# VinAIResearch/DiMSUM

Measured on AMD Instinct MI355X. Metric: denoiser-fwd latents/sec, higher is better.
Workload: dtype f32; 1 GPU; DiM-L/2 denoiser forward, 256px (4x32x32 latents, 256 tokens), 256 latents per GPU, random-init weights (reference init, zero tensors re-drawn N(0, 0.02^2)); global_batch=256, parallelism=dp1 (replicas, independent latents), launch=eager, matmul_policy=f16s (see notes.matmul_policy)

## Files before the change

### dimsum_amd/csrc/gemm_nt.hip

```cpp
#include "gemm_nt_kernel.hpp"

namespace dimsum {
namespace gemm_nt {

struct gemm_flat_t : dimsum_gemm_ext_t {
    int32_t m, n, k, operand_dtype, epilogue;
    float out_scale;
    int64_t lda, ldb, ldc;
    const void *a_ptr, *b_ptr, *bias_ptr;
    void *c_ptr;
    const void *a_inv_scale_ptr, *b_inv_scale_ptr;
};
static int gemm_flat_from(const dimsum_gemm_params_t *p, gemm_flat_t &f) {
    if (!p) return DIMSUM_ERR_NULL;
    if (p->struct_size != sizeof(dimsum_gemm_params_t)) return DIMSUM_ERR_ABI;
    const int rc = ext_from<dimsum_gemm_ext_t>(p->ext, f);
    if (rc != DIMSUM_OK) return rc;
    f.m = p->m; f.n = p->n; f.k = p->k; f.operand_dtype = p->operand_dtype; f.epilogue = p->epilogue; f.out_scale = p->out_scale;
    f.lda = p->lda; f.ldb = p->ldb; f.ldc = p->ldc;
    f.a_ptr = p->a_ptr; f.b_ptr = p->b_ptr; f.bias_ptr = p->bias_ptr; f.c_ptr = p->c_ptr;
    f.a_inv_scale_ptr = p->a_inv_scale_ptr; f.b_inv_scale_ptr = p->b_inv_scale_ptr;
    return DIMSUM_OK;
}

// ... 69 lines not shown
    if (w.probe) { *w.probe = 1; return DIMSUM_OK; }
    Args a = a0;
    a.tiles_m = a.M / 128;
    a.group_m = a.tiles_m <= 32 ? a.tiles_m : 2 * a0.group_m;
    return run<gemm_nt_m128_kernel<kOp, kEpi, kVar>>(a, a.tiles_m * a.tiles_n, 256, w);
}
inline int persist_grid() {
    int dev = 0, cus = 256;
    if (hipGetDevice(&dev) == hipSuccess) (void)hipDeviceGetAttribute(&cus, hipDeviceAttributeMultiprocessorCount, dev);
    return cus >= 8 ? cus / 8 * 8 : 8;
}
template <int kOp, int kEpi, int kVar = 0> int launch_persist(const Args &a, const Where &w) {
    if (w.probe) { *w.probe = 2; return DIMSUM_OK; }
    return run<gemm_nt_persist_kernel<kOp, kEpi, kVar>>(a, persist_grid(), 512, w);
}
template <int kEpi, int kVar = 0> int launch_f16(const Args &a, const Where &w, bool m128) {
    return m128 ? launch_m128<kOpF16, kEpi, kVar>(a, w) : launch<kOpF16, kEpi, kVar>(a, w);
}

inline bool m128_tiles(int epilogue, bool bf, int k, int tune_variant) {
    if (bf || epilogue == DIMSUM_GEMM_EPI_GATED_GELU_SPLIT3) return false;
    if (tune_variant != 0) return tune_variant == 512;
    switch (epilogue) {
        case DIMSUM_GEMM_EPI_F32: case DIMSUM_GEMM_EPI_F32_BIAS: case DIMSUM_GEMM_EPI_F16_QKV: case DIMSUM_GEMM_EPI_F32_CONV: return k <= 576;
        default: return false;
    }
}
inline bool persist_ok(const Args &a, int epilogue, bool bf, int tune_variant) {
    const bool gated = epilogue == DIMSUM_GEMM_EPI_GATED_GELU_F16;
    if (bf || tune_variant == 512 || tune_variant == 513 || !(gated || (epilogue == DIMSUM_GEMM_EPI_F32_GATE_RESIDUAL && tune_variant == 514))) return false;
    const int nk = a.K / kBK;
    return a.N % (gated ? 128 : kBN) == 0 && nk >= 4 && nk % 2 == 0 && a.tiles_m * a.tiles_n > persist_grid() && a.a_alias_tiles == 0 && a.b_alias_tiles == 0;
}

}
}

#ifdef DIMSUM_GEMM_TUNE
#define DIMSUM_GEMM_TUNE_VARIANTS(X) X(1) X(2) X(4) X(8) X(12) X(16) X(3) X(40) X(44) X(72) X(104)
#define DIMSUM_GEMM_TUNE_CASE(V) case V: return launch<kOpBf16, kEpiF32, V>(a, w);
#endif

static int gemm_nt_run(const dimsum_gemm_params_t *pub, void *stream, int *probe) {
    using namespace dimsum;
    using namespace dimsum::gemm_nt;
    gemm_flat_t p;
    Args a;
    if (const int rc = gemm_prologue(pub, p, a)) return rc;
    if (p.m <= 0 || p.n <= 0 || p.k < 2 * kBK || p.m % kBM != 0 || p.k % kBK != 0 || p.n % 4 != 0) return DIMSUM_ERR_SHAPE;
    if (p.a_alias_rows != 0 && (p.a_alias_rows < 0 || p.a_alias_rows % kBK != 0 || p.k != 3 * p.a_alias_rows)) return DIMSUM_ERR_SHAPE;
    if (p.b_alias_rows != 0 && (p.b_alias_rows < 0 || p.b_alias_rows % kBK != 0 || p.k != 3 * p.b_alias_rows || (p.epilogue != DIMSUM_GEMM_EPI_F32 && p.epilogue != DIMSUM_GEMM_EPI_F32_CONV))) return DIMSUM_ERR_SHAPE;
    if (!rows_16bit_ok(p.a_ptr, p.lda, p.a_alias_rows ? 2 * p.a_alias_rows : p.k) || !rows_16bit_ok(p.b_ptr, p.ldb, p.b_alias_rows ? 2 * p.b_alias_rows : p.k)) return DIMSUM_ERR_STRIDE;
    if (!offsets_fit(p, false, false)) return DIMSUM_ERR_STRIDE;
    a.K = p.k;
    a.a_alias_tiles = (int)(p.a_alias_rows / kBK);
    a.a_alias_from = a.a_alias_tiles;
    if (p.a_alias_weight_order) {
        if (!p.a_alias_rows) return DIMSUM_ERR_SHAPE;
        a.a_alias_tiles *= 2;
        a.a_alias_from = a.a_alias_tiles;
    }
    a.b_alias_tiles = (int)(p.b_alias_rows / kBK);
    a.stagger = p.tune_reserved > 0 ? p.tune_reserved : 0;
    if ((p.a_inv_scale_ptr == nullptr) != (p.b_inv_scale_ptr == nullptr)) return DIMSUM_ERR_NULL;
    if (a.sb && !aligned_to<char>(a.sb, 16)) return DIMSUM_ERR_STRIDE;
#ifndef DIMSUM_GEMM_TUNE
    if (p.tune_variant != 0 && p.tune_variant != 512 && p.tune_variant != 513 && p.tune_variant != 514) return DIMSUM_ERR_UNSUPPORTED;
#endif
    const bool bf = p.operand_dtype == DIMSUM_BF16;
    if (p.tune_variant == 512 && bf) return DIMSUM_ERR_UNSUPPORTED;
    const bool m128 = m128_tiles(p.epilogue, bf, p.k, p.tune_variant);
    const Where w = where(p, stream, probe);
    constexpr int kShip = kVarFullLineStores | kVarNtStores;
    if (p.epilogue == DIMSUM_GEMM_EPI_F32_GATE_RESIDUAL) {
        if (!p.residual_ptr) return DIMSUM_ERR_NULL;
        if (!rows_f32_out_ok(p) || p.residual_ld % 4 != 0 || p.residual_ld < p.n || !aligned_to<char>(p.residual_ptr, 16) ||
            (p.bias_ptr && !aligned_to<char>(p.bias_ptr, 16)) || (p.gate_ptr && (p.gate_ld % 4 != 0 || !aligned_to<char>(p.gate_ptr, 16))))
            return DIMSUM_ERR_STRIDE;
        if (p.gate_ptr && (p.rows_per_batch <= 0 || p.rows_per_batch % kBM != 0 || p.m % p.rows_per_batch != 0)) return DIMSUM_ERR_SHAPE;
        fill_right(a, p, p.n, kBN);
        a.res = reinterpret_cast<const float *>(p.residual_ptr);
        a.gate = reinterpret_cast<const float *>(p.gate_ptr);
        a.ldr = p.residual_ld; a.ldg = p.gate_ld;
        a.rows_per_batch = p.gate_ptr ? p.rows_per_batch : p.m;
        if (persist_ok(a, p.epilogue, bf, p.tune_variant)) return launch_persist<kOpF16, kEpiF32GateRes, kShip>(a, w);
        return bf ? launch<kOpBf16, kEpiF32GateRes, kShip>(a, w) : launch_f16<kEpiF32GateRes, kShip>(a, w, m128);
    }
    if (p.epilogue == DIMSUM_GEMM_EPI_F16_QKV) {
        if (bf || !a.sa || !p.gate_bound_ptr) return DIMSUM_ERR_NULL;
        if (p.rows_per_batch <= 0 || p.rows_per_batch % kBM != 0 || p.m % p.rows_per_batch != 0 || p.qkv_q_cols <= 0 || p.qkv_q_cols % 16 != 0 ||
            p.qkv_q_cols > p.n || p.n % 8 != 0)
            return DIMSUM_ERR_SHAPE;
        if (p.ldc % 8 != 0 || p.ldc < p.n || !aligned_to<char>(p.c_ptr, 16) || (p.bias_ptr && !aligned_to<char>(p.bias_ptr, 16)) ||
            (int64_t)257 * p.ldc * 2 >= ((int64_t)1 << 31))
            return DIMSUM_ERR_STRIDE;
        fill_right(a, p, p.n, kBN);
        a.gate_bound = reinterpret_cast<const float *>(p.gate_bound_ptr);
        a.rows_per_batch = p.rows_per_batch;
        a.q_cols = p.qkv_q_cols;
        return launch_f16<kEpiF16Qkv>(a, w, m128);
    }
    if (p.epilogue == DIMSUM_GEMM_EPI_GELU_F16) {
        if (bf || !a.sa || !p.gate_bound_ptr || p.a_alias_rows != 0 || p.x12_ptr || p.c_image_pieces != 0) return DIMSUM_ERR_UNSUPPORTED;
        if (!p.h_inv_scale_ptr) return DIMSUM_ERR_NULL;
        if (p.n % 8 != 0) return DIMSUM_ERR_SHAPE;
        if (p.ldc % 8 != 0 || p.ldc < p.n || !aligned_to<char>(p.c_ptr, 16) || (p.bias_ptr && !aligned_to<char>(p.bias_ptr, 16)) ||
            !aligned_to<char>(p.h_inv_scale_ptr, 4) || (int64_t)257 * p.ldc * 2 >= ((int64_t)1 << 31))
            return DIMSUM_ERR_STRIDE;
        fill_right(a, p, p.n, kBN);
        a.gate_bound = reinterpret_cast<const float *>(p.gate_bound_ptr);
        a.inv_out = reinterpret_cast<float *>(p.h_inv_scale_ptr);
        return launch_f16<kEpiGeluF16>(a, w, m128);
    }
    if (p.epilogue == DIMSUM_GEMM_EPI_F32_CONV) {
        if (!p.conv_weight_ptr) return DIMSUM_ERR_NULL;
        if (p.conv_rows <= 0 || p.conv_rows % kBM != 0 || p.conv_rows > p.m || p.conv_width < 2 || p.conv_width > 4 || p.conv_seq <= 0 || 256 % p.conv_seq != 0 ||
            p.conv_seq % 4 != 0 || p.n % p.conv_seq != 0 || p.conv_weight_ld < p.conv_width)
            return DIMSUM_ERR_SHAPE;
// ... 142 lines not shown
```

### dimsum_amd/csrc/gemm_nt_kernel.hpp

```cpp
#pragma once
#include "common.hpp"

namespace dimsum {
namespace gemm_nt {

typedef float f4 __attribute__((ext_vector_type(4)));
typedef __bf16 bf16x8_t __attribute__((ext_vector_type(8)));
typedef _Float16 f16x8_t __attribute__((ext_vector_type(8)));
typedef unsigned u32x4 __attribute__((ext_vector_type(4)));
typedef unsigned u32x2 __attribute__((ext_vector_type(2)));
typedef __attribute__((address_space(3))) void lds_void_t;
typedef __attribute__((address_space(1))) const void glb_void_t;

constexpr int kBM = 256, kBN = 256, kBK = 64;
constexpr int kHalf = 16384;
constexpr int kParity = 4 * kHalf;
constexpr int kSlotA0 = 0, kSlotA1 = kHalf, kSlotB0 = 2 * kHalf, kSlotB1 = 3 * kHalf;

enum { kOpBf16 = 0, kOpF16 = 1 };
enum { kEpiF32 = 0, kEpiGatedSplit3 = 1, kEpiGatedF16 = 2, kEpiF32Bias = 3, kEpiF32GateRes = 4, kEpiF16Qkv = 5, kEpiF32Conv = 6, kEpiGeluF16 = 7 };

struct Args {
    const char *A, *B0, *B1;
    void *C;
    const float *bias0, *bias1;
    const float *sa, *sb;
    const float *gate_bound;
    float *inv_out;
    const float *res, *gate;
    int64_t ldr, ldg;
    int rows_per_batch;
    int64_t lda, ldb, ldc;
    int M, N, K;
    int tiles_m, tiles_n;
    float out_scale;
    int group_m;
    int stagger;
    float *x12;
    int64_t ldx;
    int splits;
    int64_t c_split_stride;
    int a_alias_tiles;
    int a_alias_from;
    int tn_pieces;
    int64_t a_pair_cols, b_pair_cols;
    int b_alias_tiles;
    const float *conv_w, *conv_b;
    int conv_rows, conv_width, conv_seq, conv_w_ld;
    const float *a_block_inv;
    int a_block_inv_ld;
    const _Float16 *k_fac;
    const float *c_scale;
    const float *k_inv_a, *k_inv_b;
    int q_cols;
    int c_pieces2;
};
enum { kVarLgkmAfterBarrier = 1, kVarNoEpilogue = 2, kVarNtStores = 4, kVarFullLineStores = 8, kVarNoSetprio = 16, kVarSc1Stores = 32, kVarSc0Stores = 64, kVarKeepX12 = 128, kVarTN = 256, kVarM128 = 512, kVarRebase = 1024, kVarPersist = 2048, kVarRowFac = 4096, kVarNN = 8192 };

__device__ __forceinline__ float dpp_row_ror8(float x) {
    const int v = __builtin_bit_cast(int, x);
    return __builtin_bit_cast(float, __builtin_amdgcn_update_dpp(v, v, 0x128, 0xf, 0xf, false));
}
template <int kAux> __device__ __forceinline__ void store_f4(__amdgpu_buffer_rsrc_t rsrc, unsigned voff, const f4 &v) {
    __builtin_amdgcn_raw_buffer_store_b128(__builtin_bit_cast(u32x4, v), rsrc, voff, 0, kAux);
}

template <int kOp> __device__ __forceinline__ f4 mma(const u32x4 &a, const u32x4 &b, f4 c) {
    if constexpr (kOp == kOpBf16) return __builtin_amdgcn_mfma_f32_16x16x32_bf16(__builtin_bit_cast(bf16x8_t, a), __builtin_bit_cast(bf16x8_t, b), c, 0, 0, 0);
    else return __builtin_amdgcn_mfma_f32_16x16x32_f16(__builtin_bit_cast(f16x8_t, a), __builtin_bit_cast(f16x8_t, b), c, 0, 0, 0);
}

__device__ __forceinline__ const char *uniform_ptr(const char *q) {
    const uint64_t v = reinterpret_cast<uint64_t>(q);
    const unsigned lo = __builtin_amdgcn_readfirstlane((unsigned)v), hi = __builtin_amdgcn_readfirstlane((unsigned)(v >> 32));
    return reinterpret_cast<const char *>(((uint64_t)hi << 32) | lo);
}

__device__ __forceinline__ unsigned pick_mask(bool c) {
    unsigned m = c ? 0xffffffffu : 0u;
    asm volatile("" : "+v"(m));
    return m;
}
__device__ __forceinline__ unsigned pick_mask_lanes(bool c) {
    unsigned m = c ? 0xffffffffu : 0u;
    asm volatile("" : "+v"(m));
    return m;
}
__device__ __forceinline__ float pick(unsigned m, float a, float b) {
    return __uint_as_float((__float_as_uint(a) & m) | (__float_as_uint(b) & ~m));
}
__device__ __forceinline__ f4 pick(unsigned m, const f4 &a, const f4 &b) {
    return f4{pick(m, a[0], b[0]), pick(m, a[1], b[1]), pick(m, a[2], b[2]), pick(m, a[3], b[3])};
}

#define DIMSUM_DS_READ_B128(dst, addr, off) asm volatile("ds_read_b128 %0, %1 offset:%2" : "=v"(dst) : "v"(addr), "i"(off))
#define DIMSUM_DS_READ_TR(dst, addr, off) asm volatile("ds_read_b64_tr_b16 %0, %1 offset:%2" : "=v"(dst) : "v"(addr), "i"(off))
#define DIMSUM_WAIT_VM(n) asm volatile("s_waitcnt vmcnt(" #n ")" ::: "memory")
#ifndef DIMSUM_PERSIST_GS
#define DIMSUM_PERSIST_GS 2
#endif
#ifndef DIMSUM_EPI_PACE
#define DIMSUM_EPI_PACE 0
#endif
#define DIMSUM_STR2(x) #x
#define DIMSUM_STR(x) DIMSUM_STR2(x)
#define DIMSUM_PACE_STORES() do { if constexpr (kM1 && DIMSUM_EPI_PACE >= 0) asm volatile("s_waitcnt vmcnt(" DIMSUM_STR(DIMSUM_EPI_PACE) ")" ::: "memory"); } while (0)
#define DIMSUM_WAIT_LGKM0() asm volatile("s_waitcnt lgkmcnt(0)" ::: "memory")

__device__ __forceinline__ float gelu_tanh_f(float x) {
    const float u = 0.7978845608028654f * (x + 0.044715f * x * x * x);
    return x * fast_rcp(1.0f + fast_exp2(-2.0f * kLog2e * u));
}

template <int kOp, int kEpi, int kVar>
__device__ __forceinline__ void gemm_body(const Args &p, char *lds) {
    const unsigned lds0 = (unsigned)(uintptr_t)(__attribute__((address_space(3))) char *)lds;
    const int lane = threadIdx.x & 63;
    const int w = __builtin_amdgcn_readfirstlane(threadIdx.x >> 6);
    constexpr bool kM1 = (kVar & kVarM128) != 0;
    constexpr int kTileM = kM1 ? 128 : kBM;
    constexpr int kMiRows = kM1 ? 64 : 128;
    const int wr = kM1 ? 0 : (w >> 2), wc = w & 3;

    constexpr bool kTN = (kVar & kVarTN) != 0;
    constexpr bool kNN = (kVar & kVarNN) != 0;
    constexpr bool kBT = kTN || kNN;
    static_assert(!kBT || kEpi == kEpiF32, "the TN / NN variants have the plain fp32 epilogue");
    static_assert(!(kBT && kM1) && !(kTN && kNN), "the TN / NN variants have 256 x 256 tiles only");
    constexpr bool kPersist = (kVar & kVarPersist) != 0;
    static_assert(!kPersist || (!kTN && !kM1 && (kEpi == kEpiF32 || kEpi == kEpiF32Bias || kEpi == kEpiF32GateRes || kEpi == kEpiGatedF16)), "persistent: the 256-row NT kernel");
    int tile_m, tile_n, split = 0;
    auto map_tile = [&](int bid, int &tile_m, int &tile_n) {
        const int nwg = kPersist ? p.tiles_m * p.tiles_n : (int)gridDim.x;
        const int q = nwg >> 3, r = nwg & 7, xcd = bid & 7;
        int t = (xcd < r ? xcd * (q + 1) : r * (q + 1) + (xcd - r) * q) + (bid >> 3);
        if constexpr (kBT) {
            const int tiles = p.tiles_m * p.tiles_n;
            split = t / tiles;
            t -= split * tiles;
        }
// ... 78 lines not shown
        tn_b_tile = (int64_t)kBK * p.ldb * 2;
    }
    const unsigned st_lds = lds0 + w * 2048;
    auto stage = [&](int slot, const char *base, unsigned voff, int kt, int alias = 0) {
        const unsigned dst = st_lds + (kt & 1) * kParity + slot;
        const int src_kt = (alias && kt >= (slot < kSlotB0 ? p.a_alias_from : alias)) ? kt - alias : kt;
        const char *s = base + (int64_t)src_kt * (kBK * 2);
        __builtin_amdgcn_global_load_lds((glb_void_t *)(s + voff), (lds_void_t *)(uintptr_t)dst, 16, 0, 0);
        __builtin_amdgcn_global_load_lds((glb_void_t *)(s + 64 + voff), (lds_void_t *)(uintptr_t)(dst + 1024), 16, 0, 0);
    };
    auto stage_tn = [&](int slot, const char *base, int64_t tile_bytes, const unsigned (&voff)[2], int kt) {
        const unsigned dst = st_lds + (kt & 1) * kParity + slot;
        const char *s = base + (int64_t)kt * tile_bytes;
        __builtin_amdgcn_global_load_lds((glb_void_t *)(s + voff[0]), (lds_void_t *)(uintptr_t)dst, 16, 0, 0);
        __builtin_amdgcn_global_load_lds((glb_void_t *)(s + voff[1]), (lds_void_t *)(uintptr_t)(dst + 1024), 16, 0, 0);
    };
    auto stage_tn_a = [&](int slot, const char *base, int kt) {
        const unsigned dst = st_lds + (kt & 1) * kParity + slot;
        const int src_kt = (p.a_alias_tiles && kt >= p.a_alias_tiles) ? kt - p.a_alias_tiles : kt;
        const char *s = base + (int64_t)src_kt * tn_a_tile;
        __builtin_amdgcn_global_load_lds((glb_void_t *)(s + tn_voff_a[0]), (lds_void_t *)(uintptr_t)dst, 16, 0, 0);
        __builtin_amdgcn_global_load_lds((glb_void_t *)(s + tn_voff_a[1]), (lds_void_t *)(uintptr_t)(dst + 1024), 16, 0, 0);
    };
    auto stage_a0 = [&](int kt) { if constexpr (kTN) stage_tn_a(kSlotA0, tn_a, kt); else stage(kSlotA0, a_base, a_voff, kt, p.a_alias_tiles); };
    auto stage_a1 = [&](int kt) { if constexpr (kTN) stage_tn_a(kSlotA1, tn_a + 256, kt); else stage(kSlotA1, a_base + a_half, a_voff, kt, p.a_alias_tiles); };
    auto stage_b0 = [&](int kt) { if constexpr (kBT) stage_tn(kSlotB0, tn_b, tn_b_tile, tn_voff_b, kt); else stage(kSlotB0, b_base[0], b_voff[0], kt, p.b_alias_tiles); };
    auto stage_b1 = [&](int kt) { if constexpr (kBT) stage_tn(kSlotB1, tn_b + 256, tn_b_tile, tn_voff_b, kt); else stage(kSlotB1, b_base[1], b_voff[1], kt, p.b_alias_tiles); };
    auto stage_of = [&](const Src &s_, int which, int kt) {
        if (which == 0) stage(kSlotA0, s_.a_base, a_voff, kt, p.a_alias_tiles);
        else if (which == 1) stage(kSlotB0, s_.b_base[0], s_.b_voff[0], kt, p.b_alias_tiles);
        else if (which == 2) stage(kSlotB1, s_.b_base[1], s_.b_voff[1], kt, p.b_alias_tiles);
        else stage(kSlotA1, s_.a_base + a_half, a_voff, kt, p.a_alias_tiles);
    };

    const unsigned rd = (unsigned)((lane & 15) * 64 + (((lane >> 4) ^ (((lane >> 3) & 1) << 1)) * 16));
    const unsigned a_rd = lds0 + wr * 4 * 2048 + rd;
    const unsigned b_rd = lds0 + wc * 2 * 2048 + rd;

    unsigned a_rd_tn[4], b_rd_tn[2];
    if constexpr (kBT) {
        const int t = lane & 15, g = lane >> 4, key = ((g & 1) << 2) | (t >> 2);
        const unsigned base = lds0 + (unsigned)((4 * g + (t >> 2)) * 256 + (t & 3) * 8);
#pragma unroll
        for (int i = 0; i < 4; ++i) a_rd_tn[i] = base + (unsigned)(((wr * 4 + i) ^ key) << 5);
#pragma unroll
        for (int j = 0; j < 2; ++j) b_rd_tn[j] = base + (unsigned)(((wc * 2 + j) ^ key) << 5);
    }

    u32x4 a0[4][2], a1[4][2], b0[2][2], b1[2][2];
    f4 acc[2][2][4][2];
#pragma unroll
    for (int mi = 0; mi < 2; ++mi)
#pragma unroll
        for (int ni = 0; ni < 2; ++ni)
#pragma unroll
            for (int i = 0; i < 4; ++i)
#pragma unroll
                for (int j = 0; j < 2; ++j) acc[mi][ni][i][j] = f4{0.f, 0.f, 0.f, 0.f};

#define DIMSUM_READ_TN1(dst, addr, slot, kh)                                               \
    do {                                                                                   \
        u32x2 lo_, hi_;                                                                    \
        DIMSUM_DS_READ_TR(lo_, addr, (slot) + (kh) * 8192);                                \
        DIMSUM_DS_READ_TR(hi_, addr, (slot) + (kh) * 8192 + 4096);                         \
        dst = u32x4{lo_[0], lo_[1], hi_[0], hi_[1]};                                       \
    } while (0)
// ... 258 lines not shown
        rebase(a0, 0, (KT) + 1);                     \
        DIMSUM_PHASE_END();                                                                                                     \
    } while (0)
    bool resumed = false;
    for (;;) {
    bool has_next = false;
    int nbid = 0, ntile_m = 0, ntile_n = 0;
    Src nxt = cur;
    if constexpr (kPersist) {
        nbid = bid + (int)gridDim.x;
        has_next = nbid < p.tiles_m * p.tiles_n;
        if (has_next) {
            map_tile(nbid, ntile_m, ntile_n);
            nxt = make_src(ntile_m * kTileM, ntile_n * kTileN);
        }
    }
    if constexpr (kPersist) {
        for (int kt = 0; kt < nk; ++kt) {
            const bool own = kt + 2 < nk;
            const int skt = own ? kt + 2 : kt + 2 - nk;
            Src ss;
            ss.a_base = uniform_ptr(own ? cur.a_base : nxt.a_base);
            ss.b_base[0] = uniform_ptr(own ? cur.b_base[0] : nxt.b_base[0]);
            ss.b_base[1] = uniform_ptr(own ? cur.b_base[1] : nxt.b_base[1]);
            ss.b_voff[0] = cur.b_voff[0];
            ss.b_voff[1] = cur.b_voff[1];
            const bool w12 = !(resumed && kt < 2), w34 = !(resumed && kt < 1);
            DIMSUM_KTILE(kt, stage_of(ss, 0, skt), stage_of(ss, 1, skt), stage_of(ss, 2, skt), stage_of(ss, 3, skt), w12, w34);
        }
        if (wr == 0) __builtin_amdgcn_s_barrier();
    } else if constexpr (!kM1) {
    int kt = 0;
    for (; kt < nk - 2; ++kt) DIMSUM_KTILE(kt, stage_a0(kt + 2), stage_b0(kt + 2), stage_b1(kt + 2), stage_a1(kt + 2), true, true);
    {
        const unsigned par = (kt & 1) * kParity, par_next = kParity - par;
        DIMSUM_READ_B(b0, kSlotB0, par);
        DIMSUM_WAIT_VM(10);
        DIMSUM_PHASE_SYNC();
        DIMSUM_QUADRANT(0, 0, a0, b0);
        DIMSUM_PHASE_END();
        DIMSUM_READ_B(b1, kSlotB1, par);
        DIMSUM_WAIT_VM(8);
        DIMSUM_PHASE_SYNC();
        DIMSUM_QUADRANT(0, 1, a0, b1);
        DIMSUM_PHASE_END();
        DIMSUM_READ_A(a1, kSlotA1, par);
        read_fac(kt);
        DIMSUM_WAIT_VM(6);
        DIMSUM_PHASE_SYNC();
        rebase(a1, 1, kt);
        DIMSUM_QUADRANT(1, 1, a1, b1);
        DIMSUM_PHASE_END();
        DIMSUM_READ_A(a0, kSlotA0, par_next);
        read_fac(kt + 1);
        DIMSUM_WAIT_VM(4);
        DIMSUM_PHASE_SYNC();
        DIMSUM_QUADRANT(1, 0, a1, b0);
        rebase(a0, 0, kt + 1);
        DIMSUM_PHASE_END();
        DIMSUM_READ_B(b0, kSlotB0, par_next);
        DIMSUM_WAIT_VM(2);
        DIMSUM_PHASE_SYNC();
        DIMSUM_QUADRANT(0, 0, a0, b0);
        DIMSUM_PHASE_END();
        DIMSUM_READ_B(b1, kSlotB1, par_next);
        DIMSUM_WAIT_VM(0);
        DIMSUM_PHASE_SYNC();
        DIMSUM_QUADRANT(0, 1, a0, b1);
        DIMSUM_PHASE_END();
        DIMSUM_READ_A(a1, kSlotA1, par_next);
        read_fac(kt + 1);
        DIMSUM_PHASE_SYNC();
        rebase(a1, 1, kt + 1);
        DIMSUM_QUADRANT(1, 1, a1, b1);
        DIMSUM_PHASE_END();
        DIMSUM_QUADRANT(1, 0, a1, b0);
    }
    if (wr == 0) __builtin_amdgcn_s_barrier();
    }

    int lane_e = lane;
    if constexpr (kPersist) asm volatile("" : "+v"(lane_e));
    {
    const int lane = lane_e;
    const int ecol = wc * 32 + (lane >> 4) * 4;
    if constexpr (kVar & kVarNoEpilogue) {
#pragma unroll
        for (int mi = 0; mi < 2; ++mi)
#pragma unroll
            for (int ni = 0; ni < 2; ++ni)
#pragma unroll
                for (int i = 0; i < 4; ++i)
#pragma unroll
                    for (int j = 0; j < 2; ++j) asm volatile("" ::"v"(acc[mi][ni][i][j]));
    } else if constexpr (kEpi == kEpiF32 || kEpi == kEpiF32Bias || kEpi == kEpiF32GateRes || kEpi == kEpiF32Conv) {
        if constexpr (kEpi == kEpiF32Conv) {
            if (m0 < p.conv_rows) {
                constexpr int kNW = kM1 ? 4 : 8;
                constexpr int kHalfRows = kM1 ? 64 : 128;
                float *Ct = reinterpret_cast<float *>(p.C) + (int64_t)m0 * p.ldc + n0;
                const __amdgpu_buffer_rsrc_t crsrc = __builtin_amdgcn_make_buffer_rsrc(Ct, 0, 0x7fffffff, 0x00020000);
                const int W = p.conv_width;
                const bool has_s = p.sa != nullptr;
                const unsigned ms = pick_mask(has_s);
// ... 61 lines not shown
                }
                return;
            }
        }
        constexpr int kAux = ((kVar & kVarNtStores) ? 2 : 0) | ((kVar & kVarSc1Stores) ? 16 : 0) | ((kVar & kVarSc0Stores) ? 1 : 0);
        float *Ct = reinterpret_cast<float *>(p.C) + (int64_t)m0 * p.ldc + n0 + (kBT ? (int64_t)split * p.c_split_stride : (int64_t)0);
        const __amdgpu_buffer_rsrc_t rsrc = __builtin_amdgcn_make_buffer_rsrc(Ct, 0, 0x7fffffff, 0x00020000);
        if constexpr (kVar & kVarFullLineStores) {
            const bool up = (lane & 8) != 0;
            const int frow = wr * 64 + (lane & 7);
            const int fcol = wc * 32 + (lane >> 4) * 4 + (up ? 16 : 0);
            const bool has_s = kRebase || p.sa != nullptr;
            const unsigned ms = pick_mask(has_s);
            const bool has_sb = has_s && !kRowFac;
            const unsigned msb = pick_mask(has_sb);
            const float *sap = p.sa ? p.sa + m0 : reinterpret_cast<const float *>(p.A), *sbp = has_sb ? p.sb : reinterpret_cast<const float *>(p.B0);
            float c_scale = 1.0f;
            if constexpr (kRowFac) c_scale = p.k_inv_a ? c_scale_own : *p.c_scale;
            bool live[2];
            f4 bv[2], sbv[2], gv[2];
            auto load_cols = [&](int ni) {
                const int col = ni * 128 + fcol;
                live[ni] = n0 + col < p.N;
                const int lc = live[ni] ? n0 + col : 0;
                bv[ni] = f4{0.f, 0.f, 0.f, 0.f}; sbv[ni] = gv[ni] = f4{1.f, 1.f, 1.f, 1.f};
                if constexpr (kEpi == kEpiF32Bias) bv[ni] = *reinterpret_cast<const f4 *>(p.bias0 + lc);
                if constexpr (kEpi == kEpiF32GateRes) {
                    bv[ni] = pick(pick_mask(p.bias0 != nullptr), *reinterpret_cast<const f4 *>((p.bias0 ? p.bias0 : reinterpret_cast<const float *>(p.B0)) + lc), bv[ni]);
                    gv[ni] = pick(pick_mask(p.gate != nullptr),
                                  *reinterpret_cast<const f4 *>((p.gate ? p.gate + (int64_t)(m0 / p.rows_per_batch) * p.ldg : reinterpret_cast<const float *>(p.B0)) + lc), gv[ni]);
                }
                sbv[ni] = pick(msb, *reinterpret_cast<const f4 *>(sbp + lc), sbv[ni]);
            };
            load_cols(0);
            live[1] = n0 + 128 + fcol < p.N;
            float rs[2][4][2];
            if constexpr (!kPersist || kRebase || kEpi != kEpiF32GateRes)
#pragma unroll
            for (int mi = 0; mi < 2; ++mi)
#pragma unroll
                for (int i = 0; i < 4; ++i) {
                    const int lrow = frow + mi * kMiRows + i * 16;
                    if constexpr (kRebase) rs[mi][i][0] = rs[mi][i][1] = top[mi * 2 + (i >> 1)];
                    else if constexpr (kRowFac) {
                        rs[mi][i][0] = c_scale * pick(ms, sap[lrow], 1.0f); rs[mi][i][1] = c_scale * pick(ms, sap[lrow + 8], 1.0f);
                    }
                    else {
                        rs[mi][i][0] = pick(ms, sap[lrow], 1.0f); rs[mi][i][1] = pick(ms, sap[lrow + 8], 1.0f);
                    }
                }
            constexpr int kGS = kPersist ? DIMSUM_PERSIST_GS : 4, kNG = 16 / kGS;
            f4 rr[2][kGS][2];
            float rg[2][kGS][2];
            auto load_res = [&](int g) {
                if constexpr (kEpi == kEpiF32GateRes) {
                    const int t0 = g * kGS, ni = t0 >> 3, mi = (t0 >> 2) & 1;
                    if constexpr (kPersist) {
#pragma unroll
                        for (int k = 0; k < kGS; ++k) {
                            const int lrow = frow + mi * kMiRows + ((t0 + k) & 3) * 16;
                            rg[g & 1][k][0] = pick(ms, sap[lrow], 1.0f); rg[g & 1][k][1] = pick(ms, sap[lrow + 8], 1.0f);
                        }
                    }
                    const float *rp = p.res + (int64_t)(m0 + frow + mi * kMiRows) * p.ldr + (live[ni] ? n0 + ni * 128 + fcol : 0);
#pragma unroll
                    for (int k = 0; k < kGS; ++k) {
                        const int i = (t0 + k) & 3;
                        rr[g & 1][k][0] = *reinterpret_cast<const f4 *>(rp + (int64_t)(i * 16) * p.ldr);
                        rr[g & 1][k][1] = *reinterpret_cast<const f4 *>(rp + (int64_t)(i * 16 + 8) * p.ldr);
                    }
                }
            };
            load_res(0);
#pragma unroll
            for (int g = 0; g < kNG; ++g) {
                if (g + 1 < kNG) load_res(g + 1);
                if (g * kGS == 4) load_cols(1);
#pragma unroll
                for (int k = 0; k < kGS; ++k) {
                    const int t = g * kGS + k, ni = t >> 3, mi = (t >> 2) & 1, i = t & 3;
                    const int col = ni * 128 + fcol;
                    const f4 x0 = acc[mi][ni][i][0], x1 = acc[mi][ni][i][1];
                    f4 s0, s1;
#pragma unroll
                    for (int e = 0; e < 4; ++e) {
                        const float r0 = dpp_row_ror8(x0[e]), r1 = dpp_row_ror8(x1[e]);
                        s0[e] = up ? r1 : x0[e];
                        s1[e] = up ? x1[e] : r0;
                    }
                    const int lrow = frow + mi * kMiRows + i * 16;
                    const unsigned voff = (unsigned)((lrow * p.ldc + col) * 4);
                    constexpr bool kRowsInGroup = kPersist && kEpi == kEpiF32GateRes;
                    s0 = s0 * (sbv[ni] * (kRowsInGroup ? rg[g & 1][k][0] : rs[mi][i][0]));
                    s1 = s1 * (sbv[ni] * (kRowsInGroup ? rg[g & 1][k][1] : rs[mi][i][1]));
                    if constexpr (kEpi == kEpiF32GateRes) {
                        s0 = rr[g & 1][k][0] + gv[ni] * (s0 + bv[ni]);
                        s1 = rr[g & 1][k][1] + gv[ni] * (s1 + bv[ni]);
                    } else {
                        s0 = s0 + bv[ni];
                        s1 = s1 + bv[ni];
                    }
                    if (live[ni]) {
                        store_f4<kAux>(rsrc, voff, s0);
                        store_f4<kAux>(rsrc, voff + (unsigned)(8 * p.ldc * 4), s1);
                    }
                    if constexpr (kEpi != kEpiF32GateRes) DIMSUM_PACE_STORES();
                }
            }
        } else {
            const int frow = wr * 64 + (lane & 15);
#pragma unroll
            for (int ni = 0; ni < 2; ++ni)
#pragma unroll
                for (int j = 0; j < 2; ++j) {
                    const int col = ni * 128 + ecol + j * 16;
                    if (n0 + col < p.N) {
                        f4 bv = f4{0.f, 0.f, 0.f, 0.f};
                        if constexpr (kEpi == kEpiF32Bias) bv = *reinterpret_cast<const f4 *>(p.bias0 + n0 + col);
#pragma unroll
                        for (int mi = 0; mi < 2; ++mi)
#pragma unroll
                            for (int i = 0; i < 4; ++i)
                                store_f4<kAux>(rsrc, (unsigned)(((frow + mi * kMiRows + i * 16) * p.ldc + col) * 4), acc[mi][ni][i][j] + bv);
                    }
                }
        }
    } else if constexpr (kEpi == kEpiF16Qkv || kEpi == kEpiGeluF16) {
        constexpr bool kGelu = kEpi == kEpiGeluF16;
        constexpr int kNW = kM1 ? 4 : 8;
        float *red = reinterpret_cast<float *>(lds);
        (void)red;
        const float wl1 = p.gate_bound[0], bmax = p.gate_bound[1];
        float row_sa[2][4], row_qs[2][4];
        f4 cbv[2][2], csb[2][2];
#pragma unroll
        for (int mi = 0; mi < 2; ++mi)
#pragma unroll
            for (int i = 0; i < 4; ++i) row_sa[mi][i] = p.sa[m0 + mi * kMiRows + wr * 64 + i * 16 + (lane & 15)];
        {
            const unsigned mbias = pick_mask(p.bias0 != nullptr);
// ... 249 lines not shown
template <int kOp, int kEpi, int kVar = 0>
__global__ __launch_bounds__(512, 2) void gemm_nt_kernel(const Args p) {
    __shared__ __attribute__((aligned(1024))) char lds[2 * kParity];
    cu_stagger(p, 256);
    gemm_body<kOp, kEpi, kVar>(p, lds);
}

template <int kOp, int kEpi, int kVar = 0>
__global__ __launch_bounds__(512, 2) void gemm_nt_persist_kernel(const Args p) {
    __shared__ __attribute__((aligned(1024))) char lds[2 * kParity + 32768];
    gemm_body<kOp, kEpi, kVar | kVarPersist>(p, lds);
}

template <int kOp, int kEpi, int kVar = 0>
__global__ __launch_bounds__(512, 2) void gemm_tn_rowfac_kernel(const Args p) {
    __shared__ __attribute__((aligned(1024))) char lds[2 * kParity + 32768];
    gemm_body<kOp, kEpi, kVar | kVarRowFac>(p, lds);
}

template <int kOp, int kEpi, int kVar = 0>
__global__ __launch_bounds__(512, 2) void gemm_nn_rowfac_kernel(const Args p) {
    __shared__ __attribute__((aligned(1024))) char lds[2 * kParity + 32768];
    gemm_body<kOp, kEpi, kVar | kVarRowFac | kVarNN>(p, lds);
}

template <int kOp, int kEpi, int kVar = 0>
__global__ __launch_bounds__(256, 2) void gemm_nt_m128_kernel(const Args p) {
    __shared__ __attribute__((aligned(1024))) char lds[10 * 8192];
    cu_stagger(p, 512);
    gemm_body<kOp, kEpi, kVar | kVarM128>(p, lds);
}

#undef DIMSUM_KTILE
#undef DIMSUM_READ_A
#undef DIMSUM_READ_TN1
#undef DIMSUM_DS_READ_TR
#undef DIMSUM_READ_B
#undef DIMSUM_QUADRANT
#undef DIMSUM_PHASE_SYNC
#undef DIMSUM_PHASE_END
#undef DIMSUM_DS_READ_B128
#undef DIMSUM_DS_READ_B64
#undef DIMSUM_WAIT_VM
#undef DIMSUM_WAIT_LGKM0

}
}
```

### dimsum_amd/native.py

```python
import contextlib

import os

import torch

from . import _lib

_DT = {torch.float32: _lib.F32, torch.float16: _lib.F16, torch.bfloat16: _lib.BF16}


class _ZeroArena:
    CHUNK = 1 << 22

    def __init__(self):
        import threading
        self._lock, self._cur = threading.Lock(), {}

    def take(self, n, device):
        n = int(n)
        if n <= 0 or n > self.CHUNK // 4 or torch.cuda.is_current_stream_capturing() or os.environ.get("DIMSUM_ZERO_ARENA", "1") == "0":
            return torch.zeros(max(n, 0), device=device, dtype=torch.float32)
        pad = (n + 63) // 64 * 64
        key = (str(device), torch.cuda.current_stream(device).cuda_stream)
        with self._lock:
# ... 1491 lines not shown
            out = torch.empty((M, N), device=a.device, dtype=torch.float16)
        _check(out.dtype == torch.float16 and out.shape == (M, N) and out.stride(1) == 1, "gemm_nt: out must be (M, N) float16 rows")
    elif epilogue == "gated_f16":
        epi = _lib.GEMM_EPI_GATED_GELU_F16
        if out is None:
            out = torch.empty((M, N // 2), device=a.device, dtype=torch.float16)
        _check(out.dtype == torch.float16 and out.shape == (M, N // 2) and out.stride(1) == 1, "gemm_nt: out must be (M, F) float16 rows")
    else:
        raise ValueError(f"gemm_nt: unknown epilogue {epilogue!r}")
    h_inv = None
    if scales is not None:
        sa, sb = scales
        _gpu(sa, sb)
        _check(sa.dtype == torch.float32 and sb.dtype == torch.float32 and sa.is_contiguous() and sb.is_contiguous() and sa.numel() == M
               and sb.numel() == N, "gemm_nt: scales must be contiguous float32 (M,) and (N,)")
        if gate_bound is not None:
            _gpu(gate_bound)
            _check(epilogue in ("gated_f16", "f16_qkv", "gelu_f16") and gate_bound.dtype == torch.float32 and gate_bound.numel() == 2 and gate_bound.is_contiguous(),
                   "gemm_nt: gate_bound is a 2-element float32 tensor for the gated_f16 / f16_qkv / gelu_f16 epilogues")
            ext.update(gate_bound_ptr=_ptr(gate_bound))
            if epilogue in ("gated_f16", "gelu_f16"):
                h_inv = torch.empty((M,), device=a.device, dtype=torch.float32)
                ext.update(h_inv_scale_ptr=_ptr(h_inv))
    x12 = None
    if keep_x12:
        _check((epilogue == "gated_split3" and a.dtype == torch.bfloat16 and scales is None) or (epilogue == "gated_f16" and a.dtype == torch.float16 and h_inv is not None),
               "gemm_nt: keep_x12 goes with the gated_split3 epilogue over bf16 images or the gated_f16 epilogue over scaled-fp16 operands with gate_bound")
        x12 = torch.empty((M, N), device=a.device, dtype=torch.float32)
        ext.update(x12_ptr=_ptr(x12), x12_ld=N)
    if tune is not None:
        ext.update(tune_variant=tune[0], tune_group_m=tune[1], tune_reserved=tune[2] if len(tune) > 2 else 0)
    elif epilogue == "gated_f16" and os.environ.get("DIMSUM_GEMM_PERSIST", "1") == "0":
        ext.update(tune_variant=513)
    P = _lib.GemmParams()
    _fill_gemm(P, a, b, out, M, N, K, epi, out_scale, bias=bias, scales=scales or (None, None), events=events, **ext)
    with torch.cuda.device(a.device):
        if _gemm_kernel_log is not None:
            _gemm_kernel_log.append((epilogue if conv is None else "f32_conv", int(_lib.load().dimsum_gemm_nt_kernel_for(P))))
        _lib.check(_lib.load().dimsum_gemm_nt(P, _stream(a)), "gemm_nt")
    if x12 is not None:
        if h_inv is not None:
            return F16Image(out, h_inv), x12
        return (PairImage(out) if pair_out else out), x12
    if pair_out:
        return PairImage(out)
    return out if h_inv is None else F16Image(out, h_inv)


def xattn_supported(qkv, head_dim):
    return qkv.is_cuda and qkv.dtype == torch.float32 and qkv.stride(-1) == 1 and head_dim in (24, 32, 48, 64, 72)


def xattn_fusion_fwd(qkv1, qkv2, heads, need_lse=False, bias1=None, bias2=None, split_bf16=None, split3=False, f16s=None):
    self_attn = qkv2 is None
    if split_bf16 is None:
        split_bf16 = bool(torch.backends.cuda.matmul.allow_tf32)
    _gpu(qkv1, qkv2, bias1, bias2)
    _check(self_attn or (bias1 is None) == (bias2 is None), "xattn_fusion: pass both biases or none")
    for bb in (bias1, bias2):
        if bb is not None:
            _check(bb.dtype == torch.float32 and bb.numel() == qkv1.shape[2] and bb.is_contiguous(), "xattn_fusion: bad bias")
    B, L, W = qkv1.shape
    hd = W // (3 * heads)
    qkv_f16 = qkv1.dtype == torch.float16
    _check((qkv1.dtype == torch.float32 or (qkv_f16 and f16s is not None and bias1 is None and bias2 is None)) and qkv1.stride(2) == 1, "xattn_fusion: bad qkv")
    if not self_attn:
# ... 502 lines not shown
```

Baseline: 3499 latents/s.

## Prefetch residual tiles into LDS via DMA during GEMM tail for gate-residual epilogue

Adds a residual-DMA variant of the fp32 gate+residual GEMM epilogue. During the last k-tiles it issues global_load_lds copies of the residual tile into freed LDS slots and reads them back in the epilogue, so residual loads overlap the final MMA phases instead of being fetched afterward. It applies to f16 operands with K >= 1024 and N divisible by the tile width, and can be turned off with an env var. The risk is tighter vmcnt accounting, LDS slot reuse hazards, and extra instruction scheduling pressure in the tail.

```diff
diff --git a/dimsum_amd/csrc/gemm_nt.hip b/dimsum_amd/csrc/gemm_nt.hip
--- a/dimsum_amd/csrc/gemm_nt.hip
+++ b/dimsum_amd/csrc/gemm_nt.hip
@@ -125,6 +125,9 @@
     const int nk = a.K / kBK;
     return a.N % (gated ? 128 : kBN) == 0 && nk >= 4 && nk % 2 == 0 && a.tiles_m * a.tiles_n > persist_grid() && a.a_alias_tiles == 0 && a.b_alias_tiles == 0;
 }
+inline bool residual_dma(const Args &a, bool bf, int tune_variant) {
+    return !bf && tune_variant == 0 && a.K >= 1024 && a.N % kBN == 0 && (int64_t)17 * a.ldr * 4 < ((int64_t)1 << 31);
+}
 
 }
 }
@@ -177,6 +180,7 @@
         a.ldr = p.residual_ld; a.ldg = p.gate_ld;
         a.rows_per_batch = p.gate_ptr ? p.rows_per_batch : p.m;
         if (persist_ok(a, p.epilogue, bf, p.tune_variant)) return launch_persist<kOpF16, kEpiF32GateRes, kShip>(a, w);
+        if (residual_dma(a, bf, p.tune_variant)) return launch<kOpF16, kEpiF32GateRes, kShip | kVarResDma>(a, w);
         return bf ? launch<kOpBf16, kEpiF32GateRes, kShip>(a, w) : launch_f16<kEpiF32GateRes, kShip>(a, w, m128);
     }
     if (p.epilogue == DIMSUM_GEMM_EPI_F16_QKV) {
diff --git a/dimsum_amd/csrc/gemm_nt_kernel.hpp b/dimsum_amd/csrc/gemm_nt_kernel.hpp
--- a/dimsum_amd/csrc/gemm_nt_kernel.hpp
+++ b/dimsum_amd/csrc/gemm_nt_kernel.hpp
@@ -1,4 +1,5 @@
 #pragma once
+#include <utility>
 #include "common.hpp"
 
 namespace dimsum {
@@ -55,7 +56,7 @@
     int q_cols;
     int c_pieces2;
 };
-enum { kVarLgkmAfterBarrier = 1, kVarNoEpilogue = 2, kVarNtStores = 4, kVarFullLineStores = 8, kVarNoSetprio = 16, kVarSc1Stores = 32, kVarSc0Stores = 64, kVarKeepX12 = 128, kVarTN = 256, kVarM128 = 512, kVarRebase = 1024, kVarPersist = 2048, kVarRowFac = 4096, kVarNN = 8192 };
+enum { kVarLgkmAfterBarrier = 1, kVarNoEpilogue = 2, kVarNtStores = 4, kVarFullLineStores = 8, kVarNoSetprio = 16, kVarSc1Stores = 32, kVarSc0Stores = 64, kVarKeepX12 = 128, kVarTN = 256, kVarM128 = 512, kVarRebase = 1024, kVarPersist = 2048, kVarRowFac = 4096, kVarNN = 8192, kVarResDma = 16384 };
 
 __device__ __forceinline__ float dpp_row_ror8(float x) {
     const int v = __builtin_bit_cast(int, x);
@@ -106,6 +107,12 @@
 #define DIMSUM_STR(x) DIMSUM_STR2(x)
 #define DIMSUM_PACE_STORES() do { if constexpr (kM1 && DIMSUM_EPI_PACE >= 0) asm volatile("s_waitcnt vmcnt(" DIMSUM_STR(DIMSUM_EPI_PACE) ")" ::: "memory"); } while (0)
 #define DIMSUM_WAIT_LGKM0() asm volatile("s_waitcnt lgkmcnt(0)" ::: "memory")
+template <int kN> __device__ __forceinline__ void wait_vm() {
+    static_assert(kN >= 0 && kN <= 63, "vmcnt is a 6-bit counter");
+    asm volatile("s_waitcnt vmcnt(%0)" ::"n"(kN) : "memory");
+}
+template <class F, int... kI> __device__ __forceinline__ void for_ints(F &&f, std::integer_sequence<int, kI...>) { (f(std::integral_constant<int, kI>{}), ...); }
+template <int kN, class F> __device__ __forceinline__ void for_ints(F &&f) { for_ints(f, std::make_integer_sequence<int, kN>{}); }
 
 __device__ __forceinline__ float gelu_tanh_f(float x) {
     const float u = 0.7978845608028654f * (x + 0.044715f * x * x * x);
@@ -250,6 +257,19 @@
         else if (which == 2) stage(kSlotB1, s_.b_base[1], s_.b_voff[1], kt, p.b_alias_tiles);
         else stage(kSlotA1, s_.a_base + a_half, a_voff, kt, p.a_alias_tiles);
     };
+
+    constexpr bool kResDma = (kVar & kVarResDma) != 0;
+    static_assert(!kResDma || (kEpi == kEpiF32GateRes && (kVar & kVarFullLineStores) != 0 && (kVar & (kVarPersist | kVarM128 | kVarTN | kVarNN)) == 0),
+                  "the residual DMA serves the fp32 gate + residual epilogue of the 256-row one-tile kernel");
+    unsigned res_voff = 0;
+    auto stage_res = [&](int t, unsigned dst_off) {
+        const int ni = t >> 3, mi = (t >> 2) & 1, i = t & 3;
+        const char *s = reinterpret_cast<const char *>(p.res + (int64_t)(m0 + wr * 64 + mi * kMiRows + i * 16) * p.ldr + n0 + wc * 32 + ni * 128);
+        const unsigned dst = st_lds + dst_off;
+        __builtin_amdgcn_global_load_lds((glb_void_t *)(s + res_voff), (lds_void_t *)(uintptr_t)dst, 16, 0, 0);
+        __builtin_amdgcn_global_load_lds((glb_void_t *)(s + (int64_t)8 * p.ldr * 4 + res_voff), (lds_void_t *)(uintptr_t)(dst + 1024), 16, 0, 0);
+    };
+    (void)stage_res;
 
     const unsigned rd = (unsigned)((lane & 15) * 64 + (((lane >> 4) ^ (((lane >> 3) & 1) << 1)) * 16));
     const unsigned a_rd = lds0 + wr * 4 * 2048 + rd;
@@ -574,44 +594,55 @@
     } else if constexpr (!kM1) {
     int kt = 0;
     for (; kt < nk - 2; ++kt) DIMSUM_KTILE(kt, stage_a0(kt + 2), stage_b0(kt + 2), stage_b1(kt + 2), stage_a1(kt + 2), true, true);
+#define DIMSUM_TAIL_WAIT(T, SLOT, VM)                                                      \
+    do {                                                                                   \
+        if constexpr (kResDma) { stage_res(T, (SLOT)); DIMSUM_WAIT_VM(12); }               \
+        else DIMSUM_WAIT_VM(VM);                                                           \
+    } while (0)
     {
         const unsigned par = (kt & 1) * kParity, par_next = kParity - par;
+        if constexpr (kResDma) {
+            int lane_r = lane;
+            asm volatile("" : "+v"(lane_r));
+            res_voff = (unsigned)(((lane_r & 7) * p.ldr + (lane_r >> 4) * 4 + ((lane_r & 8) ? 16 : 0)) * 4);
+        }
         DIMSUM_READ_B(b0, kSlotB0, par);
-        DIMSUM_WAIT_VM(10);
+        DIMSUM_TAIL_WAIT(0, par + kSlotA0, 10);
         DIMSUM_PHASE_SYNC();
         DIMSUM_QUADRANT(0, 0, a0, b0);
         DIMSUM_PHASE_END();
         DIMSUM_READ_B(b1, kSlotB1, par);
-        DIMSUM_WAIT_VM(8);
+        DIMSUM_TAIL_WAIT(1, par + kSlotB0, 8);
         DIMSUM_PHASE_SYNC();
         DIMSUM_QUADRANT(0, 1, a0, b1);
         DIMSUM_PHASE_END();
         DIMSUM_READ_A(a1, kSlotA1, par);
         read_fac(kt);
-        DIMSUM_WAIT_VM(6);
+        DIMSUM_TAIL_WAIT(2, par + kSlotB1, 6);
         DIMSUM_PHASE_SYNC();
         rebase(a1, 1, kt);
         DIMSUM_QUADRANT(1, 1, a1, b1);
         DIMSUM_PHASE_END();
         DIMSUM_READ_A(a0, kSlotA0, par_next);
         read_fac(kt + 1);
-        DIMSUM_WAIT_VM(4);
+        DIMSUM_TAIL_WAIT(3, par + kSlotA1, 4);
         DIMSUM_PHASE_SYNC();
         DIMSUM_QUADRANT(1, 0, a1, b0);
         rebase(a0, 0, kt + 1);
         DIMSUM_PHASE_END();
         DIMSUM_READ_B(b0, kSlotB0, par_next);
-        DIMSUM_WAIT_VM(2);
+        DIMSUM_TAIL_WAIT(4, par_next + kSlotA0, 2);
         DIMSUM_PHASE_SYNC();
         DIMSUM_QUADRANT(0, 0, a0, b0);
         DIMSUM_PHASE_END();
         DIMSUM_READ_B(b1, kSlotB1, par_next);
-        DIMSUM_WAIT_VM(0);
+        DIMSUM_TAIL_WAIT(5, par_next + kSlotB0, 0);
         DIMSUM_PHASE_SYNC();
         DIMSUM_QUADRANT(0, 1, a0, b1);
         DIMSUM_PHASE_END();
         DIMSUM_READ_A(a1, kSlotA1, par_next);
         read_fac(kt + 1);
+        if constexpr (kResDma) stage_res(6, par_next + kSlotB1);
         DIMSUM_PHASE_SYNC();
         rebase(a1, 1, kt + 1);
         DIMSUM_QUADRANT(1, 1, a1, b1);
@@ -739,6 +770,11 @@
                 }
                 sbv[ni] = pick(msb, *reinterpret_cast<const f4 *>(sbp + lc), sbv[ni]);
             };
+            const unsigned par_tail = (unsigned)(nk & 1) * kParity;
+            if constexpr (kResDma) {
+                stage_res(7, (kParity - par_tail) + kSlotA1);
+                __builtin_amdgcn_sched_barrier(0);
+            }
             load_cols(0);
             live[1] = n0 + 128 + fcol < p.N;
             float rs[2][4][2];
@@ -756,6 +792,43 @@
                         rs[mi][i][0] = pick(ms, sap[lrow], 1.0f); rs[mi][i][1] = pick(ms, sap[lrow + 8], 1.0f);
                     }
                 }
+            if constexpr (kResDma) {
+                load_cols(1);
+                DIMSUM_WAIT_VM(0);
+                __builtin_amdgcn_sched_barrier(0);
+                const unsigned rd_lo = st_lds + (unsigned)lane * 16 + par_tail, rd_hi = st_lds + (unsigned)lane * 16 + (kParity - par_tail);
+                for_ints<16>([&](auto tc) {
+                    constexpr int t = decltype(tc)::value, ni = t >> 3, mi = (t >> 2) & 1, i = t & 3;
+                    constexpr int slot = (t & 3) == 0 ? kSlotA0 : (t & 3) == 1 ? kSlotB0 : (t & 3) == 2 ? kSlotB1 : kSlotA1;
+                    if constexpr (t >= 8) wait_vm<46 - 2 * t>();
+                    const unsigned ad = (t & 4) ? rd_hi : rd_lo;
+                    f4 r0, r1;
+                    DIMSUM_DS_READ_B128(r0, ad, slot);
+                    DIMSUM_DS_READ_B128(r1, ad, slot + 1024);
+                    DIMSUM_WAIT_LGKM0();
+                    asm volatile("" : "+v"(r0), "+v"(r1));
+                    __builtin_amdgcn_sched_barrier(0);
+                    if constexpr (t < 8) stage_res(t + 8, ((t & 4) ? kParity - par_tail : par_tail) + slot);
+                    const int col = ni * 128 + fcol;
+                    const f4 x0 = acc[mi][ni][i][0], x1 = acc[mi][ni][i][1];
+                    f4 s0, s1;
+#pragma unroll
+                    for (int e = 0; e < 4; ++e) {
+                        const float q0 = dpp_row_ror8(x0[e]), q1 = dpp_row_ror8(x1[e]);
+                        s0[e] = up ? q1 : x0[e];
+                        s1[e] = up ? x1[e] : q0;
+                    }
+                    const int lrow = frow + mi * kMiRows + i * 16;
+                    const unsigned voff = (unsigned)((lrow * p.ldc + col) * 4);
+                    s0 = s0 * (sbv[ni] * rs[mi][i][0]);
+                    s1 = s1 * (sbv[ni] * rs[mi][i][1]);
+                    s0 = r0 + gv[ni] * (s0 + bv[ni]);
+                    s1 = r1 + gv[ni] * (s1 + bv[ni]);
+                    store_f4<kAux>(rsrc, voff, s0);
+                    store_f4<kAux>(rsrc, voff + (unsigned)(8 * p.ldc * 4), s1);
+                    __builtin_amdgcn_sched_barrier(0);
+                });
+            } else {
             constexpr int kGS = kPersist ? DIMSUM_PERSIST_GS : 4, kNG = 16 / kGS;
             f4 rr[2][kGS][2];
             float rg[2][kGS][2];
@@ -813,6 +886,7 @@
                     }
                     if constexpr (kEpi != kEpiF32GateRes) DIMSUM_PACE_STORES();
                 }
+            }
             }
         } else {
             const int frow = wr * 64 + (lane & 15);
@@ -1128,6 +1202,7 @@
 }
 
 #undef DIMSUM_KTILE
+#undef DIMSUM_TAIL_WAIT
 #undef DIMSUM_READ_A
 #undef DIMSUM_READ_TN1
 #undef DIMSUM_DS_READ_TR
diff --git a/dimsum_amd/native.py b/dimsum_amd/native.py
--- a/dimsum_amd/native.py
+++ b/dimsum_amd/native.py
@@ -1547,6 +1547,8 @@
         ext.update(tune_variant=tune[0], tune_group_m=tune[1], tune_reserved=tune[2] if len(tune) > 2 else 0)
     elif epilogue == "gated_f16" and os.environ.get("DIMSUM_GEMM_PERSIST", "1") == "0":
         ext.update(tune_variant=513)
+    elif residual is not None and os.environ.get("DIMSUM_GEMM_RES_DMA", "1") == "0":
+        ext.update(tune_variant=513)
     P = _lib.GemmParams()
     _fill_gemm(P, a, b, out, M, N, K, epi, out_scale, bias=bias, scales=scales or (None, None), events=events, **ext)
     with torch.cuda.device(a.device):
```

Result: no change. 3505 latents/s (median of 2 runs) (+0.2%).
